# penn-graphics-research/claymore

Measured on AMD Instinct MI355X. Metric: particles*steps/sec, higher is better.
Workload: dtype f32

## Files before the change

### claymore_amd/_ffi.py

```python
import ctypes as C
import os

MPM_OK, MPM_ERR_INVALID, MPM_ERR_DEVICE, MPM_ERR_CAPACITY, MPM_ERR_NONFINITE, MPM_ERR_NOT_READY, MPM_ERR_INTERNAL = range(7)
J_FLUID, FIXED_COROTATED, SAND, NACC = range(4)
MATERIAL_NAMES = {"jfluid": J_FLUID, "fixed_corotated": FIXED_COROTATED, "sand": SAND, "nacc": NACC}


class Config(C.Structure):
    _fields_ = [("domain_bits", C.c_int), ("max_ppc", C.c_int), ("boundary_blocks", C.c_int),
                ("gravity", C.c_float), ("cfl", C.c_float), ("max_blocks", C.c_int64),
                ("grow", C.c_int), ("drop_overflow", C.c_int), ("sync_interval", C.c_int), ("reserved", C.c_int * 3)]


class MaterialParams(C.Structure):
    _fields_ = [("rho", C.c_float), ("volume", C.c_float), ("youngs_modulus", C.c_float),
                ("poisson_ratio", C.c_float), ("bulk", C.c_float), ("gamma", C.c_float),
                ("viscosity", C.c_float), ("beta", C.c_float), ("xi", C.c_float),
                ("cohesion", C.c_float), ("yield_surface", C.c_float), ("msqr", C.c_float),
                ("log_jp0", C.c_float), ("volume_correction", C.c_int), ("hardening_on", C.c_int),
                ("reserved", C.c_int * 5)]


class CollisionObject(C.Structure):
    _fields_ = [("type", C.c_int), ("friction", C.c_float), ("scale", C.c_float), ("dsdt", C.c_float),
# ... 49 lines not shown
}
HALO = {
    "halo_keys": (_i, [_vp, _vp, _i, _ip]),
    "halo_tag_begin": (_i, [_vp]),
    "halo_tag_peer": (_i, [_vp, _i, _vp, _i]),
    "halo_tag_end": (_i, [_vp, _ip, _ip]),
    "g2p2g_halo": (_i, [_vp, _f, _f]),
    "g2p2g_interior": (_i, [_vp, _f, _f]),
    "halo_collect": (_i, [_vp, _i, _i, _vp, _vp, _i, _ip]),
    "halo_reduce": (_i, [_vp, _i, _vp, _vp, _i]),
    "mgsp_begin": (_i, [_vp, _f, _f]),
    "mgsp_rebuild_export": (_i, [_vp, _vp, _i]),
    "mgsp_tag": (_i, [_vp, _vp, _i, _i, _i]),
    "mgsp_end": (_i, [_vp, _ip, _ip, _ip, _fp]),
}
SIGNATURES.update(HALO)
HIP_ONLY = {
    "build_info": (C.c_char_p, []),
    "last_g2p2g_ms": (_i, [_vp, _fp]),
    "streams": (_i, [_vp, _P(_vp), _P(_vp)]),
    "sync": (_i, [_vp]),
    "get_capacity": (_i, [_vp, _P(C.c_int64), _P(C.c_int64), _ip]),
    "get_diagnostics": (_i, [_vp, _P(Diagnostics)]),
    "retrieve_velocity": (_i, [_vp, _i, _vp, _vp, _vp, _P(_sz)]),
    "particle_momentum": (_i, [_vp, _i, _P(C.c_double)]),
    "checkpoint_size": (_i, [_vp, _P(_sz)]),
    "checkpoint_save": (_i, [_vp, _vp, _sz, _P(_sz)]),
    "checkpoint_load": (_i, [_vp, _vp, _sz]),
    "group_unique_id": (_i, [_vp]),
    "group_create": (_i, [_vp, _i, _i, _vp, _P(_vp)]),
    "group_create_local": (_i, [_P(_vp), _i, _P(_vp)]),
    "group_destroy": (None, [_vp]),
    "group_last_error": (C.c_char_p, [_vp]),
    "group_transport": (C.c_char_p, [_vp]),
    "group_initial_setup": (_i, [_vp]),
    "group_resume": (_i, [_vp]),
    "group_substep": (_i, [_vp, _f, _f, _fp]),
    "group_run_fixed": (_i, [_vp, _i, _f]),
    "group_compute_dt": (_f, [_vp, _f, _f, _f, _f]),
    "group_main_loop": (_i, [_vp, _i, _i, _f, _vp, _vp, _ip]),
    "group_stats": (_i, [_vp, _ip, _ip, _fp]),
    "group_retrieve_velocity": (_i, [_vp, _i, _vp, _vp, _vp, _P(_sz)]),
    "group_particle_momentum": (_i, [_vp, _i, _P(C.c_double)]),
}


# ... 32 lines not shown
```

### claymore_amd/csrc/claymore_hip.hip

```cpp
#include <hip/hip_runtime.h>

#include <algorithm>
#include <cmath>
#include <cstdio>
#include <cstdlib>
#include <chrono>
#include <cstring>
#include <string>
#include <vector>

#include "../../include/claymore_amd.h"
#include "mpm_kernels.hpp"
#include "mpm_readout.hpp"

using namespace mpm;
#define MPM_STR_(x) #x
#define MPM_STR(x) MPM_STR_(x)

namespace {
constexpr int kHaloWords	 = 128;
constexpr int kStatusBlock = ST_WORDS + kHaloWords + kMaxVelSlots * kMaxVelStride;

struct Partition {
	int* table = nullptr;
// ... 28 lines not shown

}

struct SubstepEvents {
	hipEvent_t start = nullptr, g2p2g_start = nullptr, g2p2g_end = nullptr, end = nullptr;
};

struct mpm_ctx {
	mpm_config cfg {};
	GridCfg g {};
	int device = 0;
	hipStream_t s_compute = nullptr, s_comm = nullptr;
	SubstepEvents ev;
	hipEvent_t ev_comm = nullptr, ev_halo = nullptr;
	hipEvent_t ev_tag0 = nullptr, ev_tag1 = nullptr;
	bool lean_events = false;
	hipEvent_t ev_pending = nullptr;
	hipEvent_t ev_status = nullptr;
	bool grid_preupdated = false;
	bool grid_momentum = false;
	float preupdate_dt	 = 0.f;
	float fuse_dt_once	 = 0.f;
	bool rebuild_cleared = false;
	std::vector<hipEvent_t> ev_ring;
	Partition part[2];
	float* grid[2] = {nullptr, nullptr};
	int rollid	   = 0;
	int pbc = 0, nbc = 0, ebc = 0;
	int pbc_prev = 0;
	std::vector<Model> models;
	int* d_status		  = nullptr;
	int* h_status		  = nullptr;
	unsigned* d_maxvel	  = nullptr;
	float* h_maxvel		  = nullptr;
	double* d_totals	  = nullptr;
	unsigned long long* d_counter = nullptr;
	bool ready = false;
	int capacity_events = 0;
	long long books_bias = 0;
	bool has_collision = false;
	CollisionObject collision {};
	float4* d_sdf = nullptr;
	mpm_timers timers {};
	float last_g2p2g_ms = 0.f;
	int* d_overlap	   = nullptr;
	int* d_halo_list   = nullptr;
// ... 34 lines not shown
		}                                                                                                        \
	} while(0)

static float host_maxvel(const mpm_ctx* ctx) {
	float m = 0.f;
	for(int i = 0; i < kMaxVelSlots; ++i) m = std::max(m, ctx->h_maxvel[i * kMaxVelStride]);
	return m;
}

#ifndef MPM_PAIR_BUILD
#define MPM_PAIR_BUILD 0xF
#endif
#ifndef MPM_PAIR_DEFAULT
#define MPM_PAIR_DEFAULT 0xF
#endif
static int pair_mask() {
	static const int mask = [] {
		const char* e = std::getenv("MPM_G2P2G_PAIRS");
		return (e && *e ? (int) std::strtol(e, nullptr, 0) : MPM_PAIR_DEFAULT) & MPM_PAIR_BUILD;
	}();
	return mask;
}

static int launch_prepare(mpm_ctx* ctx, int cur, int prev, bool list_is_out, int binoff_sel, const int* pbc_ptr, int nblocks_est, bool sort, bool publish);

static int fail(mpm_ctx* ctx, int code, const std::string& msg) {
	ctx->err = msg;
	return code;
}

static inline void phase_call(mpm_ctx* ctx) {
	if(ctx) ctx->group_summed = false;
}

template<typename T>
static hipError_t dalloc(T** p, size_t n) {
	return hipMalloc((void**) p, sizeof(T) * (n ? n : 1));
}

template<typename T>
struct DevScratch {
	T* p = nullptr;
	DevScratch() = default;
	DevScratch(const DevScratch&) = delete;
	DevScratch& operator=(const DevScratch&) = delete;
	~DevScratch() {
// ... 235 lines not shown
	return MPM_OK;
}

int mpm_initial_setup(mpm_ctx* ctx) {
	phase_call(ctx);
	if(!ctx || ctx->ready || ctx->models.empty()) return MPM_ERR_INVALID;
	HIP_TRY(hipSetDevice(ctx->device));
	GridCfg& g		   = ctx->g;
	hipStream_t s	   = ctx->s_compute;
	const size_t table = (size_t) g.G * g.G * g.G;
	const int r = ctx->rollid, n = r ^ 1;
	HIP_TRY(dalloc(&ctx->d_status, kStatusBlock));
	HIP_TRY(hipHostMalloc((void**) &ctx->h_status, sizeof(int) * kStatusBlock));
	memset(ctx->h_status, 0, sizeof(int) * kStatusBlock);
	ctx->d_halo_counts = ctx->d_status + ST_WORDS;
	ctx->h_halo_counts = ctx->h_status + ST_WORDS;
	ctx->d_peer_rows   = ctx->d_halo_counts + 2 + 32;
	ctx->h_peer_rows   = ctx->h_halo_counts + 2 + 32;
	ctx->d_maxvel	   = reinterpret_cast<unsigned*>(ctx->d_status + ST_WORDS + kHaloWords);
	ctx->h_maxvel	   = reinterpret_cast<float*>(ctx->h_status + ST_WORDS + kHaloWords);
	HIP_TRY(dalloc(&ctx->d_totals, 4));
	HIP_TRY(dalloc(&ctx->d_counter, 1));
	HIP_TRY(hipMemsetAsync(ctx->d_status, 0, sizeof(int) * kStatusBlock, s));
	for(int i = 0; i < 2; ++i) {
		HIP_TRY(dalloc(&ctx->part[i].table, table));
		HIP_TRY(dalloc(&ctx->part[i].count, 1));
		HIP_TRY(hipMemsetAsync(ctx->part[i].table, 0xff, sizeof(int) * table, s));
		HIP_TRY(hipMemsetAsync(ctx->part[i].count, 0, sizeof(int), s));
	}
	size_t total_particles = 0;
	for(auto& m: ctx->models) total_particles += m.n;
	size_t prov = std::min(table, total_particles + 1);
	if(ctx->cfg.max_blocks > 0) prov = std::min<size_t>(table, (size_t) ctx->cfg.max_blocks);
	Partition& P = ctx->part[n];
	HIP_TRY(dalloc(&P.keys, 3 * prov));
	g.cap = (int) prov;
	for(auto& m: ctx->models)
		if(m.n) activate_blocks_kernel<<<cdiv(m.n, 256), 256, 0, s>>>(g, m.n, m.d_xyz, P.table, P.keys, P.count, ctx->d_status);
	int pbc = 0;
	HIP_TRY(hipMemcpyAsync(&pbc, P.count, sizeof(int), hipMemcpyDeviceToHost, s));
	HIP_TRY(hipStreamSynchronize(s));
	if(pbc > g.cap) return fail(ctx, MPM_ERR_CAPACITY, "Too much active blocks: " + std::to_string(pbc));
	ctx->pbc = pbc;
	if(ctx->cfg.max_blocks <= 0 && (size_t) pbc * 27 > prov) {
		int* keys		  = nullptr;
		const size_t need = std::min(table, (size_t) pbc * 27 + 1);
// ... 180 lines not shown
	const int nwg = nblocks_ptr ? hint_blocks(ctx, nblocks) : nblocks;
#define MPM_LAUNCH_PAIR(M)                                                                                                                                                                      \
	if constexpr((MPM_PAIR_BUILD >> M) & 1) {                                                                                                                                                   \
		if(m.pair) {                                                                                                                                                                            \
			g2p2g_pair_kernel<M><<<nwg, kG2P2GThreads, 0, s>>>(ctx->g, v, cur_keys, ctx->grid[0], ctx->grid[1], block_list, only_flag, nblocks_ptr, nblocks, dt, next_dt, sk, ctx->d_status); \
			return;                                                                                                                                                                             \
		}                                                                                                                                                                                       \
	}
	switch(m.material) {
		case MPM_J_FLUID: MPM_LAUNCH_PAIR(0) break;
		case MPM_FIXED_COROTATED: MPM_LAUNCH_PAIR(1) break;
		case MPM_SAND: MPM_LAUNCH_PAIR(2) break;
		default: MPM_LAUNCH_PAIR(3) break;
	}
#undef MPM_LAUNCH_PAIR
	switch(m.material) {
		case MPM_J_FLUID: g2p2g_kernel<0><<<nwg, kG2P2GThreads, 0, s>>>(ctx->g, v, cur_keys, ctx->grid[0], ctx->grid[1], block_list, only_flag, nblocks_ptr, nblocks, dt, next_dt, sk, ctx->d_status); break;
		case MPM_FIXED_COROTATED: g2p2g_kernel<1><<<nwg, kG2P2GThreads, 0, s>>>(ctx->g, v, cur_keys, ctx->grid[0], ctx->grid[1], block_list, only_flag, nblocks_ptr, nblocks, dt, next_dt, sk, ctx->d_status); break;
		case MPM_SAND: g2p2g_kernel<2><<<nwg, kG2P2GThreads, 0, s>>>(ctx->g, v, cur_keys, ctx->grid[0], ctx->grid[1], block_list, only_flag, nblocks_ptr, nblocks, dt, next_dt, sk, ctx->d_status); break;
		default: g2p2g_kernel<3><<<nwg, kG2P2GThreads, 0, s>>>(ctx->g, v, cur_keys, ctx->grid[0], ctx->grid[1], block_list, only_flag, nblocks_ptr, nblocks, dt, next_dt, sk, ctx->d_status); break;
	}
}

static int launch_clear(mpm_ctx* ctx, int flags) {
	if((flags & kClearRebuild) && !(flags & kClearP2G)) {
		if(ctx->rebuild_cleared) flags &= ~(kClearRebuild | kClearMaxVel);
		ctx->rebuild_cleared = false;
	}
	if(!(flags & (kClearP2G | kClearRebuild))) return MPM_OK;
	ClearArgs a {};
	a.flags	  = flags;
	a.nmodels = (int) ctx->models.size();
	for(int mi = 0; mi < a.nmodels; ++mi) a.out_count[mi] = ctx->models[mi].out_count, a.keep[mi] = ctx->models[mi].keep;
	a.p2g_grid	   = ctx->grid[1];
	a.status	   = ctx->d_status;
	a.max_vel_bits = ctx->d_maxvel;
	Partition& Pn  = ctx->part[ctx->rollid ^ 1];
	a.old_table	   = Pn.table;
	a.old_keys	   = Pn.keys;
	a.old_count	   = Pn.count;
	substep_clear_kernel<<<1024, 256, 0, ctx->s_compute>>>(ctx->g, a);
	return MPM_OK;
}
static int launch_g2p2g_prologue(mpm_ctx* ctx, bool with_rebuild = false, bool fused_update = false) {
	int rc = launch_clear(ctx, with_rebuild ? (kClearP2G | kClearRebuild | (fused_update ? kClearMaxVel : 0)) : kClearP2G);
	if(rc == MPM_OK && with_rebuild) ctx->rebuild_cleared = true;
	return rc;
}

static int launch_g2p2g(mpm_ctx* ctx, float dt, float next_dt, hipEvent_t e0, hipEvent_t e1, bool with_rebuild_clear = false, bool fused_update = false) {
	hipStream_t s = ctx->s_compute;
	int rc		  = launch_g2p2g_prologue(ctx, with_rebuild_clear, fused_update);
	if(rc) return rc;
	HIP_TRY(hipEventRecord(e0, s));
	if(ctx->pbc)
		for(auto& m: ctx->models) launch_g2p2g_model(ctx, m, nullptr, &ctx->d_status[ST_PBC], ctx->pbc, dt, next_dt, s);
	HIP_TRY(hipEventRecord(e1, s));
	return MPM_OK;
}

int mpm_g2p2g(mpm_ctx* ctx, float dt, float next_dt) {
	phase_call(ctx);
	if(!ctx || !ctx->ready) return MPM_ERR_NOT_READY;
	HIP_TRY(hipSetDevice(ctx->device));
	int rc = launch_g2p2g(ctx, dt, next_dt, ctx->ev.g2p2g_start, ctx->ev.g2p2g_end);
	if(rc) return rc;
	HIP_TRY(hipGetLastError());
	HIP_TRY(hipStreamSynchronize(ctx->s_compute));
	HIP_TRY(hipEventElapsedTime(&ctx->last_g2p2g_ms, ctx->ev.g2p2g_start, ctx->ev.g2p2g_end));
	ctx->timers.g2p2g_ms = ctx->last_g2p2g_ms;
	return MPM_OK;
}

static int launch_prepare(mpm_ctx* ctx, int cur, int prev, bool list_is_out, int binoff_sel, const int* pbc_ptr, int nblocks_est, bool sort, bool publish) {
	if(nblocks_est <= 0 && !publish) return MPM_OK;
// ... 28 lines not shown
	if(fuse_dt == 0.f) fuse_dt = ctx->fuse_dt_once;
	ctx->fuse_dt_once = 0.f;
	hipStream_t s = ctx->s_compute;
	GridCfg& g	  = ctx->g;
	const int r = ctx->rollid, n = r ^ 1;
	Partition& Pn = ctx->part[n];
	Partition& Pr = ctx->part[r];
	const bool fused = fuse_dt > 0.f && !ctx->has_collision;
	ctx->grid_momentum = !fused;
	int rc			 = launch_clear(ctx, kClearRebuild | (fused ? kClearMaxVel : 0));
	if(rc) return rc;
	RebuildModels rm {};
	rm.n = (int) ctx->models.size();
	for(int mi = 0; mi < rm.n; ++mi) {
		Model& m		 = ctx->models[mi];
		rm.out_count[mi] = m.out_count;
		rm.size[mi]		 = m.size;
		rm.row_of[mi]	 = m.row_of;
		rm.binoff[mi]	 = m.binoff[r];
		rm.bin_cap[mi]	 = (long long) m.bin_cap;
	}
	int* st			  = ctx->d_status;
	const int ebc_est = std::min(g.cap, ctx->ebc + ctx->ebc / 16 + 1024);
	compact_blocks_kernel<<<std::max(1u, cdiv(ebc_est, 1024)), 1024, 0, s>>>(g, rm, Pr.keys, Pn.keys, Pn.table, st);
	const unsigned rg8 = std::max(1u, std::min(4096u, cdiv((size_t) ebc_est * 8, 256))), rg32 = std::max(1u, std::min(8192u, cdiv((size_t) ebc_est * 32, 256)));
	register_blocks_kernel<0, 1><<<rg8, 256, 0, s>>>(g, &st[ST_CNT_P], nullptr, &st[ST_CNT_N], &st[ST_PBC], Pn.table, Pn.keys, st);
	if(fused) {
		carry_grid_kernel<true><<<2048, 256, 0, s>>>(g, st, Pn.keys, Pr.table, ctx->grid[1], ctx->grid[0], fuse_dt, ctx->d_maxvel);
		ctx->grid_preupdated = true;
		ctx->preupdate_dt	 = fuse_dt;
	} else
		carry_grid_kernel<false><<<2048, 256, 0, s>>>(g, st, Pn.keys, Pr.table, ctx->grid[1], ctx->grid[0], 0.f, nullptr);
	register_blocks_kernel<-1, 1><<<rg32, 256, 0, s>>>(g, &st[ST_CNT_P], &st[ST_CNT_N], &st[ST_CNT_E], &st[ST_NBC], Pn.table, Pn.keys, st);
	if(without_prepare) return MPM_OK;
	return launch_prepare(ctx, n, r, true, n, &st[ST_CNT_P], ebc_est, true, true);
}

static int grow_capacity(mpm_ctx* ctx) {
	if(!ctx->cfg.grow) return MPM_OK;
	hipStream_t s	   = ctx->s_compute;
	const size_t table = (size_t) ctx->g.G * ctx->g.G * ctx->g.G;
	const size_t cap   = (size_t) ctx->g.cap;
	if((size_t) ctx->ebc * 4 > cap * 3 && cap < table) {
		const size_t ncap = std::min(table, cap * 3 / 2 + 1);
		HIP_TRY(hipDeviceSynchronize());
		for(int i = 0; i < 2; ++i) {
// ... 2 lines not shown
		}
		for(auto& m: ctx->models) {
			for(int i = 0; i < 2; ++i) {
				HIP_TRY(regrow(&m.binoff[i], cap + 1, ncap + 1, s));
				HIP_TRY(regrow(&m.list[i], cap * (size_t) ctx->g.ppb, ncap * (size_t) ctx->g.ppb, s));
			}
			HIP_TRY(regrow(&m.size, cap + 1, ncap + 1, s));
			HIP_TRY(regrow(&m.row_of, cap + 1, ncap + 1, s));
			HIP_TRY(regrow(&m.out_count, cap + 1, ncap + 1, s));
			HIP_TRY(regrow(&m.keep, cap + 1, ncap + 1, s));
			HIP_TRY(regrow(&m.blockinfo, cap * (size_t) kInfoRow, ncap * (size_t) kInfoRow, s));
			if(m.pair)
				for(int i = 0; i < 2; ++i) HIP_TRY(regrow(&m.pairinfo[i], (cap + 1) * (size_t) kPairChunks, (ncap + 1) * (size_t) kPairChunks, s));
		}
		if(ctx->d_overlap) {
			HIP_TRY(regrow(&ctx->d_overlap, cap + 1, ncap + 1, s));
			HIP_TRY(regrow(&ctx->d_halo_list, cap + 1, ncap + 1, s));
			HIP_TRY(regrow(&ctx->d_inner_list, cap + 1, ncap + 1, s));
		}
		for(int p = 0; p < 32; ++p)
			if(ctx->d_send_ids[p]) HIP_TRY(regrow(&ctx->d_send_ids[p], cap + 1, ncap + 1, s));
		ctx->g.cap = (int) ncap;
		ctx->capacity_events++;
	}
	for(auto& m: ctx->models) {
		const size_t need = m.n / kBin + (size_t) ctx->g.cap + 1;
		if((size_t) m.bincount * 4 > m.bin_cap * 3 || need > m.bin_cap) {
			const size_t nb = std::max(need, (size_t) m.bincount * 4 > m.bin_cap * 3 ? m.bin_cap * 3 / 2 + 1 : m.bin_cap);
			HIP_TRY(hipDeviceSynchronize());
			for(int i = 0; i < 2; ++i) HIP_TRY(regrow(&m.bins[i], m.bin_cap * m.nch * kBin, nb * m.nch * kBin, s));
			m.bin_cap = nb;
			ctx->capacity_events++;
		}
	}
	return MPM_OK;
}

static void roll_partition(mpm_ctx* ctx) {
	for(auto& m: ctx->models) m.list_in ^= 1;
	ctx->rollid ^= 1;
}

static int check_books(mpm_ctx* ctx) {
	const long long gone = (long long) ctx->h_status[ST_LOST] + (long long) ctx->h_status[ST_DROPPED] + ctx->books_bias;
	long long added = 0, held = 0;
	for(size_t mi = 0; mi < ctx->models.size(); ++mi) {
		const Model& m = ctx->models[mi];
		added += (long long) m.n;
		held += (long long) m.bucketed;
		if(gone == 0 && (long long) m.bucketed != (long long) m.n)
			return fail(ctx, MPM_ERR_INTERNAL,
						"particle books of model " + std::to_string(mi) + " do not balance: " + std::to_string(m.bucketed) + " bucketed of " + std::to_string(m.n) +
							" added, none counted as lost or dropped");
	}
	if(held + gone != added)
// ... 265 lines not shown

int mpm_get_capacity(mpm_ctx* ctx, int64_t* block_capacity, int64_t* bin_capacity, int* growth_events) {
	if(!ctx || !ctx->ready) return MPM_ERR_NOT_READY;
	if(block_capacity) *block_capacity = ctx->g.cap;
	if(bin_capacity)
		for(size_t i = 0; i < ctx->models.size() && i < 8; ++i) bin_capacity[i] = (int64_t) ctx->models[i].bin_cap;
	if(growth_events) *growth_events = ctx->capacity_events;
	return MPM_OK;
}

int mpm_get_diagnostics(mpm_ctx* ctx, mpm_diagnostics* d) {
	if(!ctx || !ctx->ready || !d) return MPM_ERR_NOT_READY;
	memset(d, 0, sizeof(*d));
	d->lost_particles = ctx->h_status[ST_LOST];
	d->discarded_p2g  = ctx->h_status[ST_ARENA];
	d->overflow_flags = ctx->h_status[ST_OVERFLOW];
	d->dropped_particles = ctx->h_status[ST_DROPPED];
#ifdef MPM_G2P2G_STATS
	for(int i = 0; i < 4; ++i) d->reserved[i] = ctx->h_status[24 + i];
#endif
	return MPM_OK;
}

int mpm_get_timers(mpm_ctx* ctx, mpm_timers* t) {
	if(!ctx || !t) return MPM_ERR_INVALID;
	*t = ctx->timers;
	return MPM_OK;
}

static int readout_particles(mpm_ctx* ctx, int model, ReadoutKind kind, float* const host[3], size_t* n) {
	HIP_TRY(hipSetDevice(ctx->device));
	hipStream_t s	 = ctx->s_compute;
	Model& m		 = ctx->models[model];
	const size_t cap = std::min(*n, m.n);
	DevScratch<float> scratch[3];
	ReadoutOut out {{m.d_xyz, nullptr, nullptr}, cap, ctx->d_counter, 0.0, nullptr};
	for(int c = 1; c < 3; ++c)
		if(host[c]) {
			HIP_TRY(scratch[c].alloc(kReadoutWidth[kind][c] * cap));
			out.col[c] = scratch[c].p;
		}
	HIP_TRY(hipMemsetAsync(ctx->d_counter, 0, sizeof(unsigned long long), s));
	if(ctx->pbc && kind == kReadState) readout_kernel<kReadState><<<ctx->pbc, kReadoutThreads, 0, s>>>(make_readout_args(ctx, m), nullptr, out);
	if(ctx->pbc && kind == kReadVelocity) readout_kernel<kReadVelocity><<<ctx->pbc, kReadoutThreads, 0, s>>>(make_readout_args(ctx, m), ctx->grid[0], out);
	HIP_TRY(hipGetLastError());
	unsigned long long count = 0;
// ... 160 lines not shown
```

### claymore_amd/csrc/mpm_checkpoint.inc

```

namespace {
struct CkptModel {
	int32_t material, nch, list_in, layout;
	int64_t n, bincount, bincount_src, bucketed;
};
struct CkptHeader {
	uint64_t magic;
	int32_t domain_bits, max_ppc, nmodels, rollid;
	int32_t pbc, nbc, ebc, prev_count;
	uint64_t total_bytes;
	uint64_t param_hash;
	int32_t prev_pbc;
	int32_t grid_velocity;
	CkptModel models[8];
};
constexpr uint64_t kCkptMagic = 0x3754504b434d504dull;

struct CkptLayout {
	size_t cur_keys, prev_keys, grid, end;
	size_t size[8], row_of[8], binoff_src[8], binoff_dst[8], bins[8], lists[8], pairinfo[8];
};
static CkptLayout ckpt_layout(const CkptHeader& h) {
	CkptLayout L {};
	size_t o	= sizeof(CkptHeader);
// ... 304 lines not shown
			if(e == hipSuccess) e = hipMemcpyAsync(d_packed, in + L.lists[mi], sizeof(int) * (size_t) M.bucketed, hipMemcpyHostToDevice, s);
			int* d_info = nullptr;
			if(e == hipSuccess && M.pair) e = dalloc(&d_info, (size_t) h.pbc * kPairChunks);
			if(e == hipSuccess && M.pair) e = hipMemcpyAsync(d_info, in + L.pairinfo[mi], sizeof(int) * (size_t) h.pbc * kPairChunks, hipMemcpyHostToDevice, s);
			if(e == hipSuccess) {
				unpack_lists_kernel<<<h.pbc, 64, 0, s>>>(ctx->g.ppb, M.size, M.row_of, d_off, M.list[M.list_in], d_packed, M.pair ? 1 : 0, M.pairinfo[0], d_info);
				e = hipGetLastError();
			}
			if(e == hipSuccess) e = hipStreamSynchronize(s);
			hipFree(d_off);
			hipFree(d_packed);
			hipFree(d_info);
			if(e != hipSuccess) return fail(ctx, MPM_ERR_DEVICE, std::string("checkpoint: ") + hipGetErrorString(e));
		}
	}
	{
		HIP_TRY(hipMemcpyAsync(ctx->h_status, ctx->d_status, sizeof(int) * ST_WORDS, hipMemcpyDeviceToHost, s));
		HIP_TRY(hipStreamSynchronize(s));
		int* st		= ctx->h_status;
		st[ST_PBC] = h.pbc, st[ST_NBC] = h.nbc, st[ST_EBC] = h.ebc, st[ST_PBCPREV] = h.prev_pbc;
		ctx->pbc_prev = h.prev_pbc;
		st[ST_CNT_P] = st[ST_CNT_N] = st[ST_CNT_E] = 0;
		st[ST_OVERFLOW] = st[ST_NONFINITE] = 0;
		for(int mi = 0; mi < kMaxModels; ++mi) {
			st[ST_BINS0 + mi]	 = mi < h.nmodels ? (int) h.models[mi].bincount : 0;
			st[ST_BINSPREV + mi] = mi < h.nmodels ? (int) h.models[mi].bincount_src : 0;
			st[ST_PART0 + mi]	 = mi < h.nmodels ? (int) h.models[mi].bucketed : 0;
		}
		{
			long long added = 0, held = 0;
			for(int mi = 0; mi < h.nmodels; ++mi) added += (long long) h.models[mi].n, held += (long long) h.models[mi].bucketed;
			ctx->books_bias = added - held - ((long long) st[ST_LOST] + (long long) st[ST_DROPPED]);
		}
		HIP_TRY(hipMemcpyAsync(ctx->d_status, st, sizeof(int) * ST_WORDS, hipMemcpyHostToDevice, s));
		HIP_TRY(hipMemsetAsync(ctx->d_maxvel, 0, sizeof(unsigned) * kMaxVelSlots * kMaxVelStride, s));
	}
	{
		int rc = launch_prepare(ctx, r, n, false, r, &ctx->d_status[ST_PBC], h.pbc, false, false);
		if(rc) return rc;
	}
	HIP_TRY(hipGetLastError());
	HIP_TRY(hipStreamSynchronize(s));
	ctx->halo_tagged = false;
	return MPM_OK;
}
```

### claymore_amd/csrc/mpm_kernels.hpp

```cpp
#pragma once
#include <hip/hip_runtime.h>
#include <type_traits>

#include "mpm_device_math.hpp"
#include "mpm_collision.hpp"

namespace mpm {

constexpr int kBin		  = 64;
constexpr int kG2P2GThreads = 64;
constexpr int kMaxModels  = 8;
constexpr int kSortKeys		= 216;
constexpr int kKeyBits		= 8;
constexpr int kStay		  = 13;

enum {
	ST_PBC = 0, ST_NBC = 1, ST_EBC = 2, ST_OVERFLOW = 3, ST_LOST = 4, ST_ARENA = 5, ST_DROPPED = 6, ST_NONFINITE = 7, ST_BINS0 = 8, ST_PART0 = 16,
	 ST_CNT_P = 29, ST_CNT_N = 30, ST_CNT_E = 31, ST_BINSPREV = 32, ST_PBCPREV = 40, ST_WORDS = 64
};

struct GridCfg {
	int G;
	int gbits;
	int ppb;
	int pid_bits;
	int boundary;
	int cap;
	float dx, dx_inv, d_inv, gravity;
};

__device__ __forceinline__ bool key_ok(const GridCfg& c, int x, int y, int z) {
	return ((unsigned) x < (unsigned) c.G) & ((unsigned) y < (unsigned) c.G) & ((unsigned) z < (unsigned) c.G);
}
__device__ __forceinline__ size_t key_index(const GridCfg& c, int x, int y, int z) {
	return ((size_t) x << (2 * c.gbits)) | ((size_t) y << c.gbits) | (size_t) z;
}
__device__ __forceinline__ int table_query(const GridCfg& c, const int* __restrict__ table, int x, int y, int z) {
	return key_ok(c, x, y, z) ? table[key_index(c, x, y, z)] : -1;
}
__device__ __forceinline__ void table_insert(const GridCfg& c, int* table, int* keys, int* count, int x, int y, int z, int* status) {
	if(!key_ok(c, x, y, z)) return;
// ... 252 lines not shown
	int n;
	int* list[kMaxModels];
	const int* size[kMaxModels];
	const int* row_of[kMaxModels];
	const int* binoff_src[kMaxModels];
	int* blockinfo[kMaxModels];
	const int* keep[kMaxModels];
	int* pairinfo[kMaxModels];
	const int* pairhand[kMaxModels];
};
template<bool SORT>
__global__ __launch_bounds__(64) void prepare_blocks_kernel(GridCfg cfg, PrepareModels pm, const int* __restrict__ pbc_ptr, const int* __restrict__ cur_table, const int* __restrict__ cur_keys, const int* __restrict__ prev_table, int* __restrict__ publish, int* __restrict__ part_count) {
	constexpr int kPrepChunk = kListChunk;
	__shared__ int s_sorted[kPairChunkMax];
	__shared__ int s_cnt[256];
	__shared__ int s_cur[256];
	const int lane = threadIdx.x;
	if(publish && blockIdx.x == 0 && lane == 0) {
		const int ebc	 = publish[ST_CNT_P] + publish[ST_CNT_N] + publish[ST_CNT_E];
		publish[ST_EBC] = ebc;
		*part_count		 = ebc;
	}
	const int pbc = min(*pbc_ptr, cfg.cap);
	for(int b = blockIdx.x; b < pbc; b += gridDim.x) {
	const int kx = cur_keys[3 * b], ky = cur_keys[3 * b + 1], kz = cur_keys[3 * b + 2];
	int size0 = 0, row0 = 0, keep0 = -2, hand0 = 0;
	if constexpr(SORT) {
		if(pm.n > 0) {
			size0 = pm.size[0][b];
			row0  = pm.row_of[0][b];
			if(pm.keep[0]) keep0 = pm.keep[0][row0];
			if(pm.pairinfo[0]) hand0 = pm.pairhand[0][(size_t) row0 * kPairChunks + (lane & (kPairChunks - 1))];
		}
	}
	int srcno = -1, other = -1;
	if(lane < 27) {
		int ox, oy, oz;
		dir_components(lane, ox, oy, oz);
		srcno = table_query(cfg, prev_table, kx + ox, ky + oy, kz + oz);
	} else if(lane < 54) {
		int ox, oy, oz;
		dir_components(lane - 27, ox, oy, oz);
		other = table_query(cfg, cur_table, kx - ox, ky - oy, kz - oz);
	} else if(lane < 62) {
		const int lb = lane - 54;
		other		 = table_query(cfg, cur_table, kx + ((lb >> 2) & 1), ky + ((lb >> 1) & 1), kz + (lb & 1));
	}
	const int key_shift		= cfg.pid_bits;
	const int tag_shift		= cfg.pid_bits + kKeyBits;
	const unsigned rec_mask = (1u << (tag_shift + 5)) - 1u;
	for(int m = 0; m < pm.n; ++m) {
		int info = other;
		if constexpr(SORT) {
		const int size = __builtin_amdgcn_readfirstlane(m == 0 ? size0 : pm.size[m][b]);
		const int row  = __builtin_amdgcn_readfirstlane(m == 0 ? row0 : pm.row_of[m][b]);
		int* list	   = pm.list[m] + (size_t) row * cfg.ppb;
		const int tail	= size & (kPrepChunk - 1);
		int* pairinfo	= pm.pairinfo[m] ? pm.pairinfo[m] + (size_t) b * kPairChunks : nullptr;
		const int kept	= m == 0 ? keep0 : (pm.keep[m] ? pm.keep[m][row] : -2);
		const bool same = pm.keep[m] && size > 0 && kept == size && (pairinfo || tail <= 64 || (tail & 63) == 0);
		constexpr int NIT = kPrepChunk / 64;
		unsigned recs[NIT];
		auto load_chunk = [&](int chunk0, int nrec) {
#pragma unroll
			for(int it = 0; it < NIT; ++it) recs[it] = (unsigned) list[chunk0 + min(it * 64 + lane, nrec - 1)];
		};
		if(size > 0 && !same) load_chunk(0, min(kPrepChunk, size));
		if(lane < 27) info = srcno >= 0 ? pm.binoff_src[m][srcno] : -1;
		auto sort_chunk = [&](int chunk0, int nrec) {
// ... 168 lines not shown
		}
		if constexpr(!SORT) {
			if(lane < 27) info = srcno >= 0 ? pm.binoff_src[m][srcno] : -1;
		}
		pm.blockinfo[m][(size_t) b * kInfoRow + lane] = info;
	}
	}
}

}
#include "mpm_g2p2g.hpp"
#include "mpm_g2p2g_pair.hpp"
namespace mpm {

struct RebuildModels {
	int n;
	const int* out_count[kMaxModels];
	int* size[kMaxModels];
	int* row_of[kMaxModels];
	int* binoff[kMaxModels];
	long long bin_cap[kMaxModels];
};

enum { kClearP2G = 1, kClearRebuild = 2, kClearMaxVel = 4 };
struct ClearArgs {
	int flags;
	int nmodels;
	int* out_count[kMaxModels];
	int* keep[kMaxModels];
	float* p2g_grid;
	int* status;
	unsigned* max_vel_bits;
	int* old_table;
	const int* old_keys;
	const int* old_count;
};
__global__ __launch_bounds__(256) void substep_clear_kernel(GridCfg cfg, ClearArgs a) {
	const int tid = blockIdx.x * 256 + threadIdx.x, nthreads = gridDim.x * 256;
	if(a.flags & kClearP2G) {
		const int nbc = min(a.status[ST_NBC], cfg.cap), ebc = min(a.status[ST_EBC], cfg.cap);
		float4* g	  = reinterpret_cast<float4*>(a.p2g_grid);
		for(int i = tid; i < nbc * 64; i += nthreads) g[i] = make_float4(0.f, 0.f, 0.f, 0.f);
		for(int m = 0; m < a.nmodels; ++m)
			for(int i = tid; i <= ebc; i += nthreads) a.out_count[m][i] = 0, a.keep[m][i] = -1;
	}
	if(a.flags & kClearRebuild) {
		const int n = min(*a.old_count, cfg.cap);
		for(int i = tid; i < n; i += nthreads) a.old_table[key_index(cfg, a.old_keys[3 * i], a.old_keys[3 * i + 1], a.old_keys[3 * i + 2])] = -1;
		if(blockIdx.x == gridDim.x - 1) {
			if(threadIdx.x < kMaxModels) {
				a.status[ST_BINSPREV + threadIdx.x] = a.status[ST_BINS0 + threadIdx.x];
				a.status[ST_BINS0 + threadIdx.x]	= 0;
				a.status[ST_PART0 + threadIdx.x]	= 0;
			}
			if(threadIdx.x >= 8 && threadIdx.x < 11) a.status[ST_CNT_P + threadIdx.x - 8] = 0;
			if(threadIdx.x == 11) a.status[ST_PBCPREV] = a.status[ST_PBC];
			if(threadIdx.x >= 64 && threadIdx.x < 64 + kMaxVelSlots) {
				unsigned* slot = a.max_vel_bits + (threadIdx.x - 64) * kMaxVelStride;
				if(*slot >= 0x7f800000u) a.status[ST_NONFINITE] = 1;
				if(a.flags & kClearMaxVel) *slot = 0u;
			}
		}
	}
}

__global__ __launch_bounds__(1024) void compact_blocks_kernel(GridCfg cfg, RebuildModels rm, const int* __restrict__ old_keys, int* __restrict__ new_keys, int* __restrict__ new_table, int* __restrict__ status) {
	__shared__ int s_part[kMaxModels];
	const int ebc = min(status[ST_EBC], cfg.cap);
	for(int b0 = blockIdx.x * blockDim.x; b0 < ebc; b0 += gridDim.x * blockDim.x) {
		const int b = b0 + threadIdx.x;
		int c[kMaxModels];
		bool any = false;
		for(int m = 0; m < rm.n; ++m) {
			c[m] = b < ebc ? rm.out_count[m][b] : 0;
			if(c[m] > cfg.ppb) {
				atomicAdd(&status[ST_DROPPED], c[m] - cfg.ppb);
				c[m] = cfg.ppb;
			}
			any |= c[m] > 0;
		}
		__syncthreads();
		if(threadIdx.x < kMaxModels) s_part[threadIdx.x] = 0;
		__syncthreads();
		for(int m = 0; m < rm.n; ++m) {
			int t = c[m];
#pragma unroll
			for(int off = 32; off > 0; off >>= 1) t += __shfl_xor(t, off);
			if((threadIdx.x & 63) == 0 && t) atomicAdd(&s_part[m], t);
		}
		__syncthreads();
		if((int) threadIdx.x < rm.n && s_part[threadIdx.x]) atomicAdd(&status[ST_PART0 + threadIdx.x], s_part[threadIdx.x]);
		const int nb = block_append(&status[ST_CNT_P], any ? 1 : 0);
		int kx = 0, ky = 0, kz = 0;
		if(any) {
			kx = old_keys[3 * b], ky = old_keys[3 * b + 1], kz = old_keys[3 * b + 2];
			new_keys[3 * nb]					  = kx;
			new_keys[3 * nb + 1]				  = ky;
			new_keys[3 * nb + 2]				  = kz;
			new_table[key_index(cfg, kx, ky, kz)] = nb;
		}
		for(int m = 0; m < rm.n; ++m) {
			const int nbins = any ? (c[m] + kBin - 1) / kBin : 0;
			const int first = block_append(&status[ST_BINS0 + m], nbins);
			if(any) {
				const bool fits = (long long) first + nbins <= rm.bin_cap[m];
				if(!fits) atomicOr(&status[ST_OVERFLOW], 4);
				rm.size[m][nb]	 = fits ? c[m] : 0;
				rm.row_of[m][nb] = b;
				rm.binoff[m][nb] = (nbins && fits) ? first : 0;
			}
		}
	}
}

template<int LO, int HI>
__global__ __launch_bounds__(256) void register_blocks_kernel(GridCfg cfg, const int* __restrict__ pbc_ptr, const int* __restrict__ base2_ptr, int* counter, int* publish, int* table, int* keys, int* status) {
	constexpr int W	   = HI - LO + 1;
	constexpr int NOFF = W * W * W;
	constexpr int LPB  = NOFF <= 8 ? 8 : 32;
	const int pbc	   = min(*pbc_ptr, cfg.cap);
	const int base	   = *pbc_ptr + (base2_ptr ? *base2_ptr : 0);
	if(publish && blockIdx.x == 0 && threadIdx.x == 0) *publish = base;
	const long long total = (long long) pbc * LPB;
	const long long bound = (total + blockDim.x - 1) / blockDim.x * blockDim.x;
	for(long long t = (long long) blockIdx.x * blockDim.x + threadIdx.x; t < bound; t += (long long) gridDim.x * blockDim.x) {
		const int b = (int) (t / LPB), o = (int) (t % LPB);
		bool claim	= false;
		int x = 0, y = 0, z = 0;
		size_t i = 0;
		if(t < total && o < NOFF) {
			x = keys[3 * b] + LO + o / (W * W);
			y = keys[3 * b + 1] + LO + (o / W) % W;
			z = keys[3 * b + 2] + LO + o % W;
			if(key_ok(cfg, x, y, z)) {
				i = key_index(cfg, x, y, z);
				if(table[i] == -1) claim = atomicCAS(&table[i], -1, -2) == -1;
			}
		}
		const int idx = base + block_append(counter, claim ? 1 : 0);
		if(claim) {
			if(idx < cfg.cap) {
				table[i]		  = idx;
				keys[3 * idx]	  = x;
				keys[3 * idx + 1] = y;
				keys[3 * idx + 2] = z;
			} else {
				table[i] = -1;
				atomicOr(&status[ST_OVERFLOW], 1);
			}
		}
	}
}

template<bool UPDATE>
__global__ __launch_bounds__(256) void carry_grid_kernel(GridCfg cfg, const int* __restrict__ status, const int* __restrict__ new_keys, const int* __restrict__ old_table, const float* __restrict__ p2g_grid, float* __restrict__ grid, float dt, unsigned* __restrict__ max_vel_bits) {
	const int nbc	  = min(status[ST_CNT_P] + status[ST_CNT_N], cfg.cap);
	const int old_nbc = min(status[ST_NBC], cfg.cap);
	const int lane = threadIdx.x & 63;
	float vel_sqr  = 0.f;
	for(int nb = blockIdx.x * 4 + (threadIdx.x >> 6); nb < nbc; nb += gridDim.x * 4) {
		const int kx = new_keys[3 * nb], ky = new_keys[3 * nb + 1], kz = new_keys[3 * nb + 2];
		const int old = table_query(cfg, old_table, kx, ky, kz);
		float4 v	  = {0.f, 0.f, 0.f, 0.f};
		if(old >= 0 && old < old_nbc) {
			const float* s = p2g_grid + (size_t) old * 256;
			v			   = {s[lane], s[64 + lane], s[128 + lane], s[192 + lane]};
		}
		if constexpr(UPDATE) {
			if(v.x > 0.0f) {
				const bool wx = kx < cfg.boundary || kx >= cfg.G - cfg.boundary;
				const bool wy = ky < cfg.boundary || ky >= cfg.G - cfg.boundary;
				const bool wz = kz < cfg.boundary || kz >= cfg.G - cfg.boundary;
				const float mass_inv = 1.f / v.x;
				const float v0		 = wx ? 0.0f : v.y * mass_inv;
				const float v1		 = (wy ? 0.0f : v.z * mass_inv) + cfg.gravity * dt;
				const float v2		 = wz ? 0.0f : v.w * mass_inv;
				v.y					 = v0;
				v.z					 = v1;
				v.w					 = v2;
				float q				 = v0 * v0 + v1 * v1 + v2 * v2;
				if(q != q) q = __builtin_inff();
				vel_sqr = fmaxf(vel_sqr, q);
			}
		}
		float* d	  = grid + (size_t) nb * 256;
// ... 180 lines not shown
```

### include/claymore_amd.h

```cpp
#ifndef CLAYMORE_AMD_H
#define CLAYMORE_AMD_H

#include <stddef.h>
#include <stdint.h>

#ifdef __cplusplus
extern "C" {
#endif

typedef enum mpm_status {
	MPM_OK			   = 0,
	MPM_ERR_INVALID	   = 1,
	MPM_ERR_DEVICE	   = 2,
	MPM_ERR_CAPACITY   = 3,
	MPM_ERR_NONFINITE  = 4,
	MPM_ERR_NOT_READY  = 5,
	MPM_ERR_INTERNAL   = 6
} mpm_status;

typedef enum mpm_material {
	MPM_J_FLUID			= 0,
	MPM_FIXED_COROTATED = 1,
	MPM_SAND			= 2,
	MPM_NACC			= 3
// ... 89 lines not shown
	float friction;
	float scale;
	float dsdt;
	float trans[3];
	float trans_vel[3];
	float omega[3];
	float rot_mat[9];
	float time;
	int reserved[3];
} mpm_collision_object;
int mpm_default_collision_object(mpm_collision_object* obj);
int mpm_set_collision_object(mpm_ctx* ctx, const mpm_collision_object* obj, const float* sdf, const float* grad_x, const float* grad_y, const float* grad_z);

int mpm_get_capacity(mpm_ctx* ctx, int64_t* block_capacity, int64_t* bin_capacity, int* growth_events);
int mpm_get_timers(mpm_ctx* ctx, mpm_timers* t);
typedef struct mpm_diagnostics {
	int64_t lost_particles;
	int64_t discarded_p2g;
	int overflow_flags;
	int dropped_particles;
	int reserved[4];
} mpm_diagnostics;
int mpm_get_diagnostics(mpm_ctx* ctx, mpm_diagnostics* d);
int mpm_grid_totals(mpm_ctx* ctx, double out[4]);
int mpm_check_table(mpm_ctx* ctx);
int mpm_dump_grid(mpm_ctx* ctx, int* keys, float* blocks, size_t* nblocks);
const char* mpm_build_info(void);
int mpm_last_g2p2g_ms(mpm_ctx* ctx, float* ms);

int mpm_test_eig(const float* F, size_t n, float* out12, int device);
int mpm_test_stress(int material, const mpm_material_params* p, const float* F, const float* logjp, size_t n, float* out19, int device);

int mpm_halo_keys(mpm_ctx* ctx, int* dev_keys, int capacity_blocks, int* count);
int mpm_halo_tag_begin(mpm_ctx* ctx);
int mpm_halo_tag_peer(mpm_ctx* ctx, int peer, const int* dev_peer_keys, int npeer_keys);
int mpm_halo_tag_end(mpm_ctx* ctx, int* halo_particle_blocks, int* send_counts);
int mpm_g2p2g_halo(mpm_ctx* ctx, float dt, float next_dt);
int mpm_g2p2g_interior(mpm_ctx* ctx, float dt, float next_dt);
int mpm_halo_collect(mpm_ctx* ctx, int peer, int gid, int* dev_keys, float* dev_blocks, int capacity_blocks, int* nsend);
int mpm_halo_reduce(mpm_ctx* ctx, int gid, const int* dev_keys, const float* dev_blocks, int nrecv);
int mpm_mgsp_begin(mpm_ctx* ctx, float dt, float next_dt);
int mpm_mgsp_rebuild_export(mpm_ctx* ctx, int* dev_keys, int pad_rows);
int mpm_mgsp_tag(mpm_ctx* ctx, const int* dev_all_keys, int pad_rows, int world, int rank);
int mpm_mgsp_end(mpm_ctx* ctx, int* send_counts, int* halo_particle_blocks, int* max_peer_rows, float* max_vel_sqr);

int mpm_streams(mpm_ctx* ctx, void** compute_stream, void** comm_stream);
// ... 24 lines not shown
```

Baseline: 34.95 billion.

## Skip partition rebuild work when the active block set is unchanged

Adds a stable-partition fast path. A verdict kernel checks whether the set of particle-occupied blocks matches the previous partition. If it does, compaction uses identity indices without atomics, the neighbor/table registration kernel returns early, carry_grid skips hash lookups, and the prepare step reads neighbor info from the previous blockinfo rows. The aim is to avoid hash-table rebuild and query costs on steps where the block set does not change. It adds an extra verdict kernel per rebuild and new correctness risks around table consistency, which capacity growth and checkpoint load guard by forcing a full rebuild.

After: 35.44 billion, median of 6. +1.4%, better.

```diff
diff --git a/claymore_amd/_ffi.py b/claymore_amd/_ffi.py
--- a/claymore_amd/_ffi.py
+++ b/claymore_amd/_ffi.py
@@ -95,6 +95,7 @@
     "sync": (_i, [_vp]),
     "get_capacity": (_i, [_vp, _P(C.c_int64), _P(C.c_int64), _ip]),
     "get_diagnostics": (_i, [_vp, _P(Diagnostics)]),
+    "stable_rebuilds": (_i, [_vp, _P(C.c_int64)]),
     "retrieve_velocity": (_i, [_vp, _i, _vp, _vp, _vp, _P(_sz)]),
     "particle_momentum": (_i, [_vp, _i, _P(C.c_double)]),
     "checkpoint_size": (_i, [_vp, _P(_sz)]),
diff --git a/claymore_amd/csrc/claymore_hip.hip b/claymore_amd/csrc/claymore_hip.hip
--- a/claymore_amd/csrc/claymore_hip.hip
+++ b/claymore_amd/csrc/claymore_hip.hip
@@ -74,6 +74,8 @@
 	float preupdate_dt	 = 0.f;
 	float fuse_dt_once	 = 0.f;
 	bool rebuild_cleared = false;
+	bool force_full_rebuild = false;
+	bool verdict_pending	= false;
 	std::vector<hipEvent_t> ev_ring;
 	Partition part[2];
 	float* grid[2] = {nullptr, nullptr};
@@ -154,6 +156,14 @@
 	return mask;
 }
 
+static bool stable_partition() {
+	static const bool on = [] {
+		const char* e = std::getenv("MPM_STABLE_PARTITION");
+		return !(e && e[0] == '0');
+	}();
+	return on;
+}
+
 static int launch_prepare(mpm_ctx* ctx, int cur, int prev, bool list_is_out, int binoff_sel, const int* pbc_ptr, int nblocks_est, bool sort, bool publish);
 
 static int fail(mpm_ctx* ctx, int code, const std::string& msg) {
@@ -435,6 +445,8 @@
 	HIP_TRY(dalloc(&ctx->d_totals, 4));
 	HIP_TRY(dalloc(&ctx->d_counter, 1));
 	HIP_TRY(hipMemsetAsync(ctx->d_status, 0, sizeof(int) * kStatusBlock, s));
+	ctx->h_status[ST_BLOCKSET] = 1;
+	HIP_TRY(hipMemcpyAsync(&ctx->d_status[ST_BLOCKSET], &ctx->h_status[ST_BLOCKSET], sizeof(int), hipMemcpyHostToDevice, s));
 	for(int i = 0; i < 2; ++i) {
 		HIP_TRY(dalloc(&ctx->part[i].table, table));
 		HIP_TRY(dalloc(&ctx->part[i].count, 1));
@@ -661,12 +673,17 @@
 	}
 }
 
-static int launch_clear(mpm_ctx* ctx, int flags) {
+static int launch_clear(mpm_ctx* ctx, int flags, bool stable = false) {
 	if((flags & kClearRebuild) && !(flags & kClearP2G)) {
 		if(ctx->rebuild_cleared) flags &= ~(kClearRebuild | kClearMaxVel);
 		ctx->rebuild_cleared = false;
 	}
 	if(!(flags & (kClearP2G | kClearRebuild))) return MPM_OK;
+	if(flags & kClearP2G) {
+		if(!stable || !stable_partition() || ctx->force_full_rebuild) flags |= kClearFullRebuild;
+		ctx->verdict_pending	= !(flags & kClearFullRebuild);
+		ctx->force_full_rebuild = false;
+	}
 	ClearArgs a {};
 	a.flags	  = flags;
 	a.nmodels = (int) ctx->models.size();
@@ -681,15 +698,15 @@
 	substep_clear_kernel<<<1024, 256, 0, ctx->s_compute>>>(ctx->g, a);
 	return MPM_OK;
 }
-static int launch_g2p2g_prologue(mpm_ctx* ctx, bool with_rebuild = false, bool fused_update = false) {
-	int rc = launch_clear(ctx, with_rebuild ? (kClearP2G | kClearRebuild | (fused_update ? kClearMaxVel : 0)) : kClearP2G);
+static int launch_g2p2g_prologue(mpm_ctx* ctx, bool with_rebuild = false, bool fused_update = false, bool stable = false) {
+	int rc = launch_clear(ctx, with_rebuild ? (kClearP2G | kClearRebuild | (fused_update ? kClearMaxVel : 0)) : kClearP2G, stable);
 	if(rc == MPM_OK && with_rebuild) ctx->rebuild_cleared = true;
 	return rc;
 }
 
 static int launch_g2p2g(mpm_ctx* ctx, float dt, float next_dt, hipEvent_t e0, hipEvent_t e1, bool with_rebuild_clear = false, bool fused_update = false) {
 	hipStream_t s = ctx->s_compute;
-	int rc		  = launch_g2p2g_prologue(ctx, with_rebuild_clear, fused_update);
+	int rc		  = launch_g2p2g_prologue(ctx, with_rebuild_clear, fused_update, true);
 	if(rc) return rc;
 	HIP_TRY(hipEventRecord(e0, s));
 	if(ctx->pbc)
@@ -764,6 +781,9 @@
 	}
 	int* st			  = ctx->d_status;
 	const int ebc_est = std::min(g.cap, ctx->ebc + ctx->ebc / 16 + 1024);
+	if(ctx->verdict_pending)
+		blockset_verdict_kernel<<<std::max(1u, std::min(1024u, cdiv(ebc_est, 256))), 256, 0, s>>>(g, rm, st);
+	ctx->verdict_pending = false;
 	compact_blocks_kernel<<<std::max(1u, cdiv(ebc_est, 1024)), 1024, 0, s>>>(g, rm, Pr.keys, Pn.keys, Pn.table, st);
 	const unsigned rg8 = std::max(1u, std::min(4096u, cdiv((size_t) ebc_est * 8, 256))), rg32 = std::max(1u, std::min(8192u, cdiv((size_t) ebc_est * 32, 256)));
 	register_blocks_kernel<0, 1><<<rg8, 256, 0, s>>>(g, &st[ST_CNT_P], nullptr, &st[ST_CNT_N], &st[ST_PBC], Pn.table, Pn.keys, st);
@@ -812,6 +832,7 @@
 			if(ctx->d_send_ids[p]) HIP_TRY(regrow(&ctx->d_send_ids[p], cap + 1, ncap + 1, s));
 		ctx->g.cap = (int) ncap;
 		ctx->capacity_events++;
+		ctx->force_full_rebuild = true;
 	}
 	for(auto& m: ctx->models) {
 		const size_t need = m.n / kBin + (size_t) ctx->g.cap + 1;
@@ -821,6 +842,7 @@
 			for(int i = 0; i < 2; ++i) HIP_TRY(regrow(&m.bins[i], m.bin_cap * m.nch * kBin, nb * m.nch * kBin, s));
 			m.bin_cap = nb;
 			ctx->capacity_events++;
+			ctx->force_full_rebuild = true;
 		}
 	}
 	return MPM_OK;
@@ -1132,6 +1154,12 @@
 	return MPM_OK;
 }
 
+int mpm_stable_rebuilds(mpm_ctx* ctx, int64_t* count) {
+	if(!ctx || !ctx->ready || !count) return MPM_ERR_NOT_READY;
+	*count = ctx->h_status[ST_STABLE];
+	return MPM_OK;
+}
+
 int mpm_get_timers(mpm_ctx* ctx, mpm_timers* t) {
 	if(!ctx || !t) return MPM_ERR_INVALID;
 	*t = ctx->timers;
diff --git a/claymore_amd/csrc/mpm_checkpoint.inc b/claymore_amd/csrc/mpm_checkpoint.inc
--- a/claymore_amd/csrc/mpm_checkpoint.inc
+++ b/claymore_amd/csrc/mpm_checkpoint.inc
@@ -350,6 +350,7 @@
 		ctx->pbc_prev = h.prev_pbc;
 		st[ST_CNT_P] = st[ST_CNT_N] = st[ST_CNT_E] = 0;
 		st[ST_OVERFLOW] = st[ST_NONFINITE] = 0;
+		st[ST_BLOCKSET] = 1;
 		for(int mi = 0; mi < kMaxModels; ++mi) {
 			st[ST_BINS0 + mi]	 = mi < h.nmodels ? (int) h.models[mi].bincount : 0;
 			st[ST_BINSPREV + mi] = mi < h.nmodels ? (int) h.models[mi].bincount_src : 0;
@@ -370,5 +371,6 @@
 	HIP_TRY(hipGetLastError());
 	HIP_TRY(hipStreamSynchronize(s));
 	ctx->halo_tagged = false;
+	ctx->force_full_rebuild = true;
 	return MPM_OK;
 }
diff --git a/claymore_amd/csrc/mpm_kernels.hpp b/claymore_amd/csrc/mpm_kernels.hpp
--- a/claymore_amd/csrc/mpm_kernels.hpp
+++ b/claymore_amd/csrc/mpm_kernels.hpp
@@ -16,7 +16,8 @@
 
 enum {
 	ST_PBC = 0, ST_NBC = 1, ST_EBC = 2, ST_OVERFLOW = 3, ST_LOST = 4, ST_ARENA = 5, ST_DROPPED = 6, ST_NONFINITE = 7, ST_BINS0 = 8, ST_PART0 = 16,
-	 ST_CNT_P = 29, ST_CNT_N = 30, ST_CNT_E = 31, ST_BINSPREV = 32, ST_PBCPREV = 40, ST_WORDS = 64
+	 ST_CNT_P = 29, ST_CNT_N = 30, ST_CNT_E = 31, ST_BINSPREV = 32, ST_PBCPREV = 40,
+	ST_BLOCKSET = 42, ST_STABLE = 43, ST_WORDS = 64
 };
 
 struct GridCfg {
@@ -315,6 +316,7 @@
 		*part_count		 = ebc;
 	}
 	const int pbc = min(*pbc_ptr, cfg.cap);
+	const bool identity = publish && publish[ST_BLOCKSET] == 0;
 	for(int b = blockIdx.x; b < pbc; b += gridDim.x) {
 	const int kx = cur_keys[3 * b], ky = cur_keys[3 * b + 1], kz = cur_keys[3 * b + 2];
 	int size0 = 0, row0 = 0, keep0 = -2, hand0 = 0;
@@ -327,17 +329,20 @@
 		}
 	}
 	int srcno = -1, other = -1;
-	if(lane < 27) {
-		int ox, oy, oz;
-		dir_components(lane, ox, oy, oz);
-		srcno = table_query(cfg, prev_table, kx + ox, ky + oy, kz + oz);
-	} else if(lane < 54) {
-		int ox, oy, oz;
-		dir_components(lane - 27, ox, oy, oz);
-		other = table_query(cfg, cur_table, kx - ox, ky - oy, kz - oz);
-	} else if(lane < 62) {
-		const int lb = lane - 54;
-		other		 = table_query(cfg, cur_table, kx + ((lb >> 2) & 1), ky + ((lb >> 1) & 1), kz + (lb & 1));
+	{
+		int ox = 0, oy = 0, oz = 0;
+		if(lane < 27)
+			dir_components(lane, ox, oy, oz);
+		else if(lane < 54)
+			dir_components(lane - 27, ox, oy, oz), ox = -ox, oy = -oy, oz = -oz;
+		else if(lane < 62)
+			ox = ((lane - 54) >> 2) & 1, oy = ((lane - 54) >> 1) & 1, oz = (lane - 54) & 1;
+		const int* p = identity ? pm.blockinfo[0] + (size_t) b * kInfoRow + (lane < 27 ? 53 - lane : lane) : (lane < 27 ? prev_table : cur_table) + key_index(cfg, kx + ox, ky + oy, kz + oz);
+		const int v	 = lane < 62 && (identity || key_ok(cfg, kx + ox, ky + oy, kz + oz)) ? *p : -1;
+		if(lane < 27)
+			srcno = v;
+		else
+			other = v;
 	}
 	const int key_shift		= cfg.pid_bits;
 	const int tag_shift		= cfg.pid_bits + kKeyBits;
@@ -552,7 +557,7 @@
 	long long bin_cap[kMaxModels];
 };
 
-enum { kClearP2G = 1, kClearRebuild = 2, kClearMaxVel = 4 };
+enum { kClearP2G = 1, kClearRebuild = 2, kClearMaxVel = 4, kClearFullRebuild = 8 };
 struct ClearArgs {
 	int flags;
 	int nmodels;
@@ -573,6 +578,7 @@
 		for(int i = tid; i < nbc * 64; i += nthreads) g[i] = make_float4(0.f, 0.f, 0.f, 0.f);
 		for(int m = 0; m < a.nmodels; ++m)
 			for(int i = tid; i <= ebc; i += nthreads) a.out_count[m][i] = 0, a.keep[m][i] = -1;
+		if(tid == 0) a.status[ST_BLOCKSET] = (a.flags & kClearFullRebuild) ? 1 : 0;
 	}
 	if(a.flags & kClearRebuild) {
 		const int n = min(*a.old_count, cfg.cap);
@@ -594,9 +600,28 @@
 	}
 }
 
+__global__ __launch_bounds__(256) void blockset_verdict_kernel(GridCfg cfg, RebuildModels rm, int* __restrict__ status) {
+	const int pbc = min(status[ST_PBC], cfg.cap), ebc = min(status[ST_EBC], cfg.cap);
+	bool diff = false;
+	for(int b = blockIdx.x * 256 + threadIdx.x; b < ebc; b += gridDim.x * 256) {
+		bool any = false;
+		for(int m = 0; m < rm.n; ++m) any |= rm.out_count[m][b] > 0;
+		diff |= any != (b < pbc);
+	}
+	if(__any(diff) && (threadIdx.x & 63) == 0) status[ST_BLOCKSET] = 1;
+}
+
 __global__ __launch_bounds__(1024) void compact_blocks_kernel(GridCfg cfg, RebuildModels rm, const int* __restrict__ old_keys, int* __restrict__ new_keys, int* __restrict__ new_table, int* __restrict__ status) {
 	__shared__ int s_part[kMaxModels];
-	const int ebc = min(status[ST_EBC], cfg.cap);
+	const int ebc		= min(status[ST_EBC], cfg.cap);
+	const bool identity = status[ST_BLOCKSET] == 0;
+	if(identity && blockIdx.x == 0 && threadIdx.x == 0) {
+		const int pbc = status[ST_PBC], nbc = status[ST_NBC];
+		status[ST_CNT_P] = pbc;
+		status[ST_CNT_N] = nbc - pbc;
+		status[ST_CNT_E] = status[ST_EBC] - nbc;
+		status[ST_STABLE] += 1;
+	}
 	for(int b0 = blockIdx.x * blockDim.x; b0 < ebc; b0 += gridDim.x * blockDim.x) {
 		const int b = b0 + threadIdx.x;
 		int c[kMaxModels];
@@ -620,9 +645,9 @@
 		}
 		__syncthreads();
 		if((int) threadIdx.x < rm.n && s_part[threadIdx.x]) atomicAdd(&status[ST_PART0 + threadIdx.x], s_part[threadIdx.x]);
-		const int nb = block_append(&status[ST_CNT_P], any ? 1 : 0);
+		const int nb = identity ? b : block_append(&status[ST_CNT_P], any ? 1 : 0);
 		int kx = 0, ky = 0, kz = 0;
-		if(any) {
+		if(identity ? b < ebc : any) {
 			kx = old_keys[3 * b], ky = old_keys[3 * b + 1], kz = old_keys[3 * b + 2];
 			new_keys[3 * nb]					  = kx;
 			new_keys[3 * nb + 1]				  = ky;
@@ -651,6 +676,7 @@
 	const int pbc	   = min(*pbc_ptr, cfg.cap);
 	const int base	   = *pbc_ptr + (base2_ptr ? *base2_ptr : 0);
 	if(publish && blockIdx.x == 0 && threadIdx.x == 0) *publish = base;
+	if(status[ST_BLOCKSET] == 0) return;
 	const long long total = (long long) pbc * LPB;
 	const long long bound = (total + blockDim.x - 1) / blockDim.x * blockDim.x;
 	for(long long t = (long long) blockIdx.x * blockDim.x + threadIdx.x; t < bound; t += (long long) gridDim.x * blockDim.x) {
@@ -686,11 +712,12 @@
 __global__ __launch_bounds__(256) void carry_grid_kernel(GridCfg cfg, const int* __restrict__ status, const int* __restrict__ new_keys, const int* __restrict__ old_table, const float* __restrict__ p2g_grid, float* __restrict__ grid, float dt, unsigned* __restrict__ max_vel_bits) {
 	const int nbc	  = min(status[ST_CNT_P] + status[ST_CNT_N], cfg.cap);
 	const int old_nbc = min(status[ST_NBC], cfg.cap);
+	const bool identity = status[ST_BLOCKSET] == 0;
 	const int lane = threadIdx.x & 63;
 	float vel_sqr  = 0.f;
 	for(int nb = blockIdx.x * 4 + (threadIdx.x >> 6); nb < nbc; nb += gridDim.x * 4) {
 		const int kx = new_keys[3 * nb], ky = new_keys[3 * nb + 1], kz = new_keys[3 * nb + 2];
-		const int old = table_query(cfg, old_table, kx, ky, kz);
+		const int old = identity ? nb : table_query(cfg, old_table, kx, ky, kz);
 		float4 v	  = {0.f, 0.f, 0.f, 0.f};
 		if(old >= 0 && old < old_nbc) {
 			const float* s = p2g_grid + (size_t) old * 256;
diff --git a/include/claymore_amd.h b/include/claymore_amd.h
--- a/include/claymore_amd.h
+++ b/include/claymore_amd.h
@@ -135,6 +135,7 @@
 	int reserved[4];
 } mpm_diagnostics;
 int mpm_get_diagnostics(mpm_ctx* ctx, mpm_diagnostics* d);
+int mpm_stable_rebuilds(mpm_ctx* ctx, int64_t* count);
 int mpm_grid_totals(mpm_ctx* ctx, double out[4]);
 int mpm_check_table(mpm_ctx* ctx);
 int mpm_dump_grid(mpm_ctx* ctx, int* keys, float* blocks, size_t* nblocks);
```
